# lc700x/desktop2stereo

Measured on AMD Instinct MI355X. Metric: stereo frames/sec @1080p DepthAnything-v2-ViT-B, higher is better.
Workload: dtype bf16; 1 GPU; DepthAnything-v2-vitb bf16, 1920x1080 uint8 RGB noise frames, batch 1 per GPU, Depth Resolution 518 (model input 294x518), Full-SBS uint8 output 3840x1080, pred; parallelism=frame-sharded dp1, no data-path collective (each rank generates its own frames)

## Files before the change

### desktop2stereo_amd/csrc/conv3.hip

```cpp
#include "conv3_tile.h"
#include <algorithm>

namespace d2s {

static_assert(sizeof(GemmA) + sizeof(GemmEpi) + 8 >= KERNARG_WARM_BYTES, "KERNARG_WARM reads past the kernarg segment");


template <int N_> __device__ __forceinline__ void c3_wait_vm() { asm volatile("s_waitcnt vmcnt(%0) lgkmcnt(0)" ::"n"(N_) : "memory"); }

template <int PST> __device__ __forceinline__ int c3_lane_pixel(int fr) {
    if constexpr ((PST & 1) == 0) return fr;
    else return fr < 4 ? 2 * fr : (fr < 12 ? 2 * (fr - 4) + 1 : 2 * (fr - 8));
}
template <int PST> __device__ __forceinline__ int c3_chunk_slot(int c) {
    if constexpr ((PST & 1) == 0) return c;
    else return (c & ~3) | ((c & 1) << 1) | ((c >> 1) & 1);
}

template <int CPP, int PST, int BN, int WM, int WN, int NS, int HG = 3 >
__global__ void __launch_bounds__(64 * WM * WN)
conv3_halo2_kernel(GemmA a, const bf16_t* __restrict__ W, int M, int N, int Kpad, GemmEpi e, int xn) {
    KERNARG_WARM(kaw_)
    KERNARG_WARM_END(kaw_)
    constexpr int TW = 16, TH = 8, HWD = TW + 2, HPX = (TH + 2) * HWD;
// ... 631 lines not shown
        c3_load_wfrags<64>(wf, W, N, Kpad, 0, fr, fg);
        c3_head_consts(e, N, fg, cb, cw);
        __syncthreads();
        int tn = walk.at(++kk);
        __syncthreads();
        const int cw4 = wid * 4;
        const int hb0 = (cw4 * HWD + fr) * PST + fg;
        int buf = 0;
        for (; t >= 0;) {
            f32x4 acc[4][2];
            const u32x4* hp = lds + buf * HALO + hb0;
            auto mma_rows = [&](auto r0c) {
                constexpr int R0 = decltype(r0c)::value;
                static_for<3>([&](auto rc) {
                    constexpr int r = R0 + decltype(rc)::value;
                    static_for<3>([&](auto kxc) {
                        constexpr int kx = decltype(kxc)::value;
#pragma unroll
                        for (int ks = 0; ks < 2; ++ks) {
                            const u32x4 fa = hp[(r * HWD + kx) * PST + ks * 4];
                            static_for<3>([&](auto kyc) {
                                constexpr int ky = 2 - decltype(kyc)::value;
                                constexpr int i = r - ky;
                                if constexpr (i >= 0 && i < 4) {
#pragma unroll
                                    for (int j = 0; j < 2; ++j) mma_chunk(acc[i][j], wf[ky * 3 + kx][ks][j], fa, bf16_t());
                                }
                            });
                        }
                    });
                });
            };
#pragma unroll
            for (int i = 0; i < 4; ++i)
#pragma unroll
                for (int j = 0; j < 2; ++j) acc[i][j] = (f32x4){0.f, 0.f, 0.f, 0.f};
            C3U_T(u0)
            mma_rows(std::integral_constant<int, 0>());
            C3U_T(u1)
            __syncthreads();
            C3U_T(u2)
            const int tnn = tn >= 0 ? walk.at(++kk) : -1;
            mma_rows(std::integral_constant<int, 3>());
            int b, ty0, tx0;
            tiles.org(t, b, ty0, tx0);
            float sr[4];
#pragma unroll
            for (int i = 0; i < 4; ++i) {
                float s = 0.f;
#pragma unroll
                for (int j = 0; j < 2; ++j) s += c3_head_dot(acc[i][j], cb[j], cw[j]);
                sr[i] = s;
            }
            typedef unsigned u2_ __attribute__((ext_vector_type(2)));
            const u2_ p01 = __builtin_amdgcn_permlane16_swap(__float_as_uint(sr[0]), __float_as_uint(sr[1]), false, false);
            const u2_ p23 = __builtin_amdgcn_permlane16_swap(__float_as_uint(sr[2]), __float_as_uint(sr[3]), false, false);
            const float c01 = __uint_as_float(p01[0]) + __uint_as_float(p01[1]);
            const float c23 = __uint_as_float(p23[0]) + __uint_as_float(p23[1]);
            const u2_ q = __builtin_amdgcn_permlane32_swap(__float_as_uint(c01), __float_as_uint(c23), false, false);
            const float sv = __uint_as_float(q[0]) + __uint_as_float(q[1]);
            {
                const int y = ty0 + cw4 + fg, x = tx0 + fr;
                if (y < a.Ho && x < a.Wo) ((float*)e.out)[((long)b * a.Ho + y) * a.Wo + x] = head_activation(sv + e.head_b3, e.head_max_depth);
            }
            if (VS < VU && tn >= 0) v_pass(tile_geo(tn), buf ^ 1, KS_(), KU_());
            C3U_T(u3)
            __syncthreads();
            C3U_T(u4)
            C3U_ACC(0, u1 - u0) C3U_ACC(1, u2 - u1) C3U_ACC(2, u3 - u2) C3U_ACC(3, u4 - u3) C3U_ACC(8, 1)
            buf ^= 1;
            t = tn; tn = tnn;
        }
    } else {
        TileGeo gn = tile_geo(t), gnn = gn;
        h_request(gn);
        h_compute();
        __syncthreads();
        int tn = walk.at(++kk);
        v_pass(gn, 0, K0_(), KU_());
        if (tn >= 0) { gn = tile_geo(tn); h_request(gn); }
        __syncthreads();
        int buf = 0;
        for (; t >= 0;) {
            C3U_T(u0)
            if (tn >= 0) h_compute();
            C3U_T(u1)
            __syncthreads();
            C3U_T(u2)
            const int tnn = tn >= 0 ? walk.at(++kk) : -1;
            if (tn >= 0) {
                if (tnn >= 0) { gnn = tile_geo(tnn); h_request(gnn); }
                v_pass(gn, buf ^ 1, K0_(), KS_());
                gn = gnn;
            }
            C3U_T(u3)
            __syncthreads();
            C3U_T(u4)
            C3U_ACC(4, u1 - u0) C3U_ACC(5, u2 - u1) C3U_ACC(6, u3 - u2) C3U_ACC(7, u4 - u3)
            buf ^= 1;
            t = tn; tn = tnn;
        }
    }
}

#ifdef D2S_C3_TIMING
__device__ unsigned long long c3_timing[256 * 8];
#define C3_T(var) const long var = wall_clock64();
#define C3_ACC(SLOT, expr) { if (threadIdx.x == 0 && blockIdx.x < 256) c3_timing[blockIdx.x * 8 + (SLOT)] += (unsigned long long)(expr); }
#else
#define C3_T(var) {}
#define C3_ACC(SLOT, expr) {}
#endif

template <int TH, int TW>
__global__ void __launch_bounds__(512)
conv3_wide_kernel(GemmA a, const bf16_t* __restrict__ W, int N, int Kpad, GemmEpi e, int ntiles) {
    KERNARG_WARM(kaw_)
    KERNARG_WARM_END(kaw_)
    constexpr int CPP = 16, PST = 17, HWD = TW + 2, HPX = (TH + 2) * HWD, HALO = HPX * PST;
    constexpr int NCH = HPX * CPP, NLD = (NCH + 511) / 512;
    constexpr int WN = 2, FM = 4, FN = 4, FPR = TW / 16;
    constexpr int NS = 8, WST = 128 * 4, NKT = 36, PD = NS - 1;
    constexpr int HKT = 28;
    static_assert(TH * TW == 256 && TW % 16 == 0, "256-pixel tiles of 16-pixel fragments");
    __shared__ __attribute__((aligned(16))) u32x4 lds[NS * WST + HALO];
    D2S_POISON_LDS(lds, NS * WST + HALO)
    u32x4* const halo = lds + NS * WST;

    const int tid = threadIdx.x, lane = tid & 63;
    const int wid = __builtin_amdgcn_readfirstlane(tid >> 6);
    const int wave_m = wid / WN, wave_n = wid % WN, grp = wid >> 2;
    const int fr = lane & 15, fg = lane >> 4, px = c3_lane_pixel<PST>(fr);
    const C3Tiles<TH, TW> tiles(a);
    const C3Walk<true> walk(ntiles);
    int kk = 0, t = walk.at(0);
    if (t < 0) return;

    const __amdgpu_buffer_rsrc_t rsW = __builtin_amdgcn_make_buffer_rsrc(uniform_ptr(W), 0, (unsigned)((long)((N + 255) / 256 * 256) * Kpad * 2), 0x00020000);
    auto wswz = [](int r) { const int k = (r >> 2) & 3; return (((k ^ (k >> 1)) & 1) << 1) | (k >> 1); };
    unsigned voW;
    {
        const int r = wid * 16 + (lane >> 2);
        voW = (unsigned)((long)r * Kpad * 2) + (unsigned)(((lane & 3) ^ wswz(r)) * 16);
    }
    auto issue_w = [&](int stage, int kt) { lds_dma16(rsW, lds + stage * WST + wid * 64, voW, kt * 64); };

    const int floor_ = relu_floor_bf16(a);
    u32x4 hr[NLD];
    auto load_halo = [&](int tt) {
        int b, ty0, tx0;
        tiles.org(tt, b, ty0, tx0);
        const bf16_t* img = (const bf16_t*)a.ptr + (long)b * a.Hi * a.Wi * a.C;
#pragma unroll
        for (int k = 0; k < NLD; ++k) {
            const int idx = tid + k * 512;
            const int p = idx >> 4, c = idx & 15;
            const int hy = p / HWD, hx = p - hy * HWD;
            int iy = ty0 + hy - 1, ix = tx0 + hx - 1;
            const bool in = idx < NCH && iy >= 0 && iy < a.Hi && ix >= 0 && ix < a.Wi;
            iy = in ? iy : 0; ix = in ? ix : 0;
            const u32x4 v = *(const u32x4*)(img + ((long)iy * a.Wi + ix) * a.C + c * 8);
            hr[k] = in ? v : (u32x4){0u, 0u, 0u, 0u};
        }
    };
    auto store_halo = [&]() {
#pragma unroll
        for (int k = 0; k < NLD; ++k) {
            const int idx = tid + k * 512;
            if (idx < NCH) halo[(idx >> 4) * PST + c3_chunk_slot<PST>(idx & 15)] = relu_frag(hr[k], floor_, bf16_t());
        }
    };

    const u32x4* hb[FM];
    int frow[FM], fcol[FM];
#pragma unroll
    for (int i = 0; i < FM; ++i) {
        const int f = wave_m * FM + i;
        frow[i] = f / FPR; fcol[i] = (f % FPR) * 16 + px;
        hb[i] = halo + (frow[i] * HWD + fcol[i]) * PST + c3_chunk_slot<PST>(fg);
    }
    int wro[FN];
#pragma unroll
    for (int jn = 0; jn < FN; ++jn) { const int r = wave_n * 64 + jn * 16 + fr; wro[jn] = r * 4 + (fg ^ wswz(r)); }

#pragma unroll
    for (int k = 0; k < PD - 1; ++k) issue_w(k, k);
    load_halo(t);
    store_halo();
    int gb = 0;
    C3_T(t_begin)
    while (t >= 0) {
        C3_T(t_a)
        const int tn = walk.at(++kk);
        const int tl = tn >= 0 ? tn : t;
        f32x4 acc[FM][FN];
#pragma unroll
        for (int i = 0; i < FM; ++i)
#pragma unroll
            for (int jn = 0; jn < FN; ++jn) acc[i][jn] = (f32x4){0.f, 0.f, 0.f, 0.f};
        u32x4 fa[2][FM], fb[2][FN];
        auto read_frags = [&](auto ktc, u32x4* fa_, u32x4* fb_) {
            constexpr int kt = decltype(ktc)::value;
            constexpr int tap = kt / 4, q = kt % 4, ky = tap / 3, kx = tap % 3;
            const u32x4* B_l = lds + ((gb + kt) & (NS - 1)) * WST;
#pragma unroll
            for (int jn = 0; jn < FN; ++jn) fb_[jn] = B_l[wro[jn]];
#pragma unroll
            for (int i = 0; i < FM; ++i) fa_[i] = hb[i][(ky * HWD + kx) * PST + q * 4];
        };
        c3_wait_vm<0>();
        __builtin_amdgcn_s_barrier();
        issue_w((gb + PD - 1) & (NS - 1), PD - 1);
        read_frags(std::integral_constant<int, 0>{}, fa[0], fb[0]);
        if (grp) __builtin_amdgcn_s_barrier();
        static_for<NKT>([&](auto ktc) {
            constexpr int kt = decltype(ktc)::value;
            __builtin_amdgcn_sched_barrier(0);
#pragma unroll
            for (int i = 0; i < FM; ++i)
#pragma unroll
                for (int jn = 0; jn < FN; ++jn) mma_chunk(acc[i][jn], fb[kt & 1][jn], fa[kt & 1][i], bf16_t());
            __builtin_amdgcn_sched_barrier(0);
            __builtin_amdgcn_s_barrier();
            if constexpr (kt < NKT - 1) {
                issue_w((gb + kt + PD) & (NS - 1), (kt + PD) % NKT);
                if constexpr (kt == HKT) load_halo(tl);
                read_frags(std::integral_constant<int, kt + 1>{}, fa[(kt + 1) & 1], fb[(kt + 1) & 1]);
                if constexpr (kt + 2 < NKT) {
                    if constexpr (kt >= HKT && kt <= HKT + PD - 2) asm volatile("s_waitcnt vmcnt(%0)" ::"n"(NLD + PD - 2) : "memory");
                    else asm volatile("s_waitcnt vmcnt(%0)" ::"n"(PD - 2) : "memory");
                }
            }
            __builtin_amdgcn_sched_barrier(0);
            __builtin_amdgcn_s_barrier();
#ifdef D2S_C3_TIMING
            if constexpr (kt == 0) { C3_ACC(4, wall_clock64() - t_a) }
#endif
        });
        if (!grp) __builtin_amdgcn_s_barrier();
        C3_T(t_b)
        C3_ACC(0, t_b - t_a)
        int b, ty0, tx0;
        tiles.org(t, b, ty0, tx0);
        bool ok[FM];
        long mo[FM];
        uint2 rr[FM][FN];
#pragma unroll
        for (int i = 0; i < FM; ++i) {
            const int y = ty0 + frow[i], x = tx0 + fcol[i];
            ok[i] = y < a.Ho && x < a.Wo;
            mo[i] = ok[i] ? ((long)(b * a.Ho + y) * a.Wo + x) * e.ldc + wave_n * 64 + fg * 4 : (long)(wave_n * 64 + fg * 4);
        }
        auto load_res = [&]() {
            const bf16_t* rp = (const bf16_t*)e.res1;
#pragma unroll
            for (int i = 0; i < FM; ++i)
#pragma unroll
                for (int jn = 0; jn < FN; ++jn) rr[i][jn] = *(const uint2*)(rp + mo[i] + jn * 16);
        };
        float cb[FN][4];
#pragma unroll
        for (int jn = 0; jn < FN; ++jn) {
            if (e.bias) load4(e.bias + wave_n * 64 + jn * 16 + fg * 4, cb[jn]);
            else cb[jn][0] = cb[jn][1] = cb[jn][2] = cb[jn][3] = 0.f;
        }
        if (e.res1) load_res();
        C3_T(t_c)
        C3_ACC(1, t_c - t_b)
        __builtin_amdgcn_s_waitcnt(0xc07f);
        __builtin_amdgcn_s_barrier();
        if (tn >= 0) store_halo();
        C3_T(t_d)
        C3_ACC(2, t_d - t_c)
#pragma unroll
        for (int i = 0; i < FM; ++i)
#pragma unroll
            for (int jn = 0; jn < FN; ++jn) {
                float v[4] = {acc[i][jn][0] + cb[jn][0], acc[i][jn][1] + cb[jn][1], acc[i][jn][2] + cb[jn][2], acc[i][jn][3] + cb[jn][3]};
                if (e.act == ACT_RELU) { v[0] = fmaxf(v[0], 0.f); v[1] = fmaxf(v[1], 0.f); v[2] = fmaxf(v[2], 0.f); v[3] = fmaxf(v[3], 0.f); }
                if (e.res1) {
                    const uint2 r = rr[i][jn];
                    v[0] += __uint_as_float(r.x << 16); v[1] += __uint_as_float(r.x & 0xffff0000u);
                    v[2] += __uint_as_float(r.y << 16); v[3] += __uint_as_float(r.y & 0xffff0000u);
                }
                if (ok[i]) *(uint2*)((bf16_t*)e.out + mo[i] + jn * 16) = make_uint2(pk_bf16(v[0], v[1]), pk_bf16(v[2], v[3]));
            }
        C3_ACC(6, wall_clock64() - t_d)
        C3_ACC(3, 1)
        gb = (gb + NKT) & (NS - 1); t = tn;
    }
    c3_wait_vm<0>();
    C3_ACC(5, wall_clock64() - t_begin)
}


struct RcuArgs {
    const bf16_t* x;
    bf16_t* out;
    const bf16_t *w1, *w2, *wp;
    const float *b1, *b2, *bp;
    int H, W, nimg, Kpad, KpadP;
};
constexpr int RCU_TH = 4, RCU_TW = 8;
typedef short s16x4 __attribute__((ext_vector_type(4)));
__device__ __forceinline__ uint2 rcu_pack4(const float v[4], bool relu) {
    uint2 t = make_uint2(pk_bf16(v[0], v[1]), pk_bf16(v[2], v[3]));
    if (relu) t = __builtin_bit_cast(uint2, __builtin_elementwise_max(__builtin_bit_cast(s16x4, t), (s16x4){0, 0, 0, 0}));
    return t;
}
typedef unsigned int u32x2 __attribute__((ext_vector_type(2)));
__device__ __forceinline__ void rcu_lds_write_b64(const u32x4* chunk, int half, uint2 v) {
    const unsigned addr = (unsigned)(unsigned long)((__attribute__((address_space(3))) const char*)chunk) + (unsigned)half * 8u;
    const u32x2 d = {v.x, v.y};
    asm volatile("ds_write_b64 %0, %1" ::"v"(addr), "v"(d) : "memory");
}
template <int PROJ>
__global__ void __launch_bounds__(512)
conv3_rcu_kernel(RcuArgs r) {
    constexpr int TH = RCU_TH, TW = RCU_TW, CPP = 16, PST = 17, NW = 8;
    constexpr int W0 = TW + 4, P0 = (TH + 4) * W0;
    constexpr int W1 = TW + 2, P1 = (TH + 2) * W1;
    constexpr int NKT = 18, NG = 2 * NKT + (PROJ ? 2 : 0);
    constexpr int WST = 128 * 8;
    constexpr int NS = 7, PD = NS - 1, BI = 128 / (8 * NW);
    static_assert(P1 <= 64 && TH * TW == 32 && BI == 2 && NG > PD, "fragment counts below are for a 4 x 8 tile");
    __shared__ __attribute__((aligned(16))) u32x4 lds[NS * WST + P0 * PST + P1 * PST];
    D2S_POISON_LDS(lds, NS * WST + P0 * PST + P1 * PST)
    u32x4* const h0 = lds + NS * WST;
    u32x4* const h1 = h0 + P0 * PST;
    u32x4* const h2 = h0;

    const int tid = threadIdx.x, lane = tid & 63;
    const int wid = __builtin_amdgcn_readfirstlane(tid >> 6);
    const int fr = lane & 15, fg = lane >> 4;
    GemmA a = {};
    a.ptr = r.x; a.Hi = a.Ho = r.H; a.Wi = a.Wo = r.W; a.C = 128; a.relu = 1;
    const C3Tiles<TH, TW> tiles(a);
    int b, ty0, tx0;
    tiles.org(blockIdx.x, b, ty0, tx0);

    const int n0 = wid * 16 + fg * 4;
    float c1[4], c2[4], cp[4] = {0.f, 0.f, 0.f, 0.f};
    load4(r.b1 + n0, c1); load4(r.b2 + n0, c2);
    if constexpr (PROJ) load4(r.bp + n0, cp);

    const unsigned wbytes = 256u * (unsigned)r.Kpad * 2u, pbytes = 256u * (unsigned)r.KpadP * 2u;
    const __amdgpu_buffer_rsrc_t rs1 = __builtin_amdgcn_make_buffer_rsrc(uniform_ptr(r.w1), 0, wbytes, 0x00020000);
    const __amdgpu_buffer_rsrc_t rs2 = __builtin_amdgcn_make_buffer_rsrc(uniform_ptr(r.w2), 0, wbytes, 0x00020000);
    const __amdgpu_buffer_rsrc_t rsP = __builtin_amdgcn_make_buffer_rsrc(uniform_ptr(PROJ ? r.wp : r.w2), 0, PROJ ? pbytes : wbytes, 0x00020000);
    unsigned voW[BI], voP[BI];
#pragma unroll
    for (int i = 0; i < BI; ++i) {
        const int row = (i * NW + wid) * 8 + (lane >> 3);
        const unsigned ch = (unsigned)(((lane & 7) ^ ((row >> 1) & 7)) * 16);
        voW[i] = (unsigned)(row * r.Kpad * 2) + ch;
        voP[i] = (unsigned)(row * r.KpadP * 2) + ch;
    }
    auto issue = [&](int g, int slot) {
        u32x4* st_ = lds + slot * WST;
        if (g < NKT) {
#pragma unroll
            for (int i = 0; i < BI; ++i) lds_dma16(rs1, st_ + (i * NW + wid) * 64, voW[i], g * 128);
        } else if (!PROJ || g < 2 * NKT) {
#pragma unroll
            for (int i = 0; i < BI; ++i) lds_dma16(rs2, st_ + (i * NW + wid) * 64, voW[i], (g - NKT) * 128);
        } else {
#pragma unroll
            for (int i = 0; i < BI; ++i) lds_dma16(rsP, st_ + (i * NW + wid) * 64, voP[i], (g - 2 * NKT) * 128);
        }
    };
#pragma unroll
    for (int t = 0; t < PD; ++t) issue(t, t);

    conv_halo_fill<bf16_t, 64 * NW, 3>(a, b, ty0 - 1, tx0 - 1, W0, P0, CPP, tid, h0,
        [&](int p, int c) { return p * PST + c; },
        [&](u32x4 v) { return relu_frag(v, relu_floor_bf16(a), bf16_t()); });
#pragma unroll
    for (int q = 0; q < 4; ++q) asm volatile("" : "+v"(c1[q]), "+v"(c2[q]), "+v"(cp[q]));

    int g = 0, slot = 0, islot = PD;
    auto ring_step = [&]() -> const u32x4* {
        const int rem = NG - 1 - g;
        if (rem >= PD - 1) c3_wait_vm<(PD - 1) * BI>();
        else if (rem == 4) c3_wait_vm<4 * BI>();
        else if (rem == 3) c3_wait_vm<3 * BI>();
        else if (rem == 2) c3_wait_vm<2 * BI>();
        else if (rem == 1) c3_wait_vm<1 * BI>();
        else c3_wait_vm<0>();
        __builtin_amdgcn_s_barrier();
        if (g + PD < NG) issue(g + PD, islot);
        const u32x4* B_l = lds + slot * WST;
        ++g;
        slot = slot + 1 == NS ? 0 : slot + 1;
        islot = islot + 1 == NS ? 0 : islot + 1;
        return B_l;
    };
    static_assert(PD == 6, "ring_step spells out the waits of the last PD - 1 tiles");
    int wo[2];
    {
        const int row = wid * 16 + fr;
#pragma unroll
        for (int ks = 0; ks < 2; ++ks) wo[ks] = row * 8 + ((ks * 4 + fg) ^ ((row >> 1) & 7));
    }

    {
        const u32x4* hb[4];
#pragma unroll
        for (int f = 0; f < 4; ++f) {
            const int p = f * 16 + fr < P1 ? f * 16 + fr : P1 - 1;
            hb[f] = h0 + ((p / W1) * W0 + p % W1) * PST + fg;
        }
        f32x4 acc[4];
#pragma unroll
        for (int f = 0; f < 4; ++f) acc[f] = (f32x4){0.f, 0.f, 0.f, 0.f};
#pragma unroll 1
        for (int kt = 0; kt < NKT; ++kt) {
            const int tap = kt >> 1, ky = (tap * 11) >> 5, kx = tap - 3 * ky;
            const int toff = (ky * W0 + kx) * PST + (kt & 1) * 8;
            const u32x4* B_l = ring_step();
            u32x4 fb[2], fa[2][4];
#pragma unroll
            for (int ks = 0; ks < 2; ++ks) {
                fb[ks] = B_l[wo[ks]];
#pragma unroll
                for (int f = 0; f < 4; ++f) fa[ks][f] = hb[f][toff + ks * 4];
            }
            __builtin_amdgcn_sched_barrier(0);
#pragma unroll
            for (int ks = 0; ks < 2; ++ks)
#pragma unroll
                for (int f = 0; f < 4; ++f) mma_chunk(acc[f], fb[ks], fa[ks][f], bf16_t());
        }
#pragma unroll
        for (int f = 0; f < 4; ++f) {
            const int p = f * 16 + fr;
            const int py = p / W1, px = p - py * W1;
            const int iy = ty0 - 1 + py, ix = tx0 - 1 + px;
            const float v[4] = {acc[f][0] + c1[0], acc[f][1] + c1[1], acc[f][2] + c1[2], acc[f][3] + c1[3]};
            uint2 t = rcu_pack4(v, true);
            if (!(iy >= 0 && iy < r.H && ix >= 0 && ix < r.W)) t = make_uint2(0u, 0u);
            if (p < P1) rcu_lds_write_b64(h1 + p * PST + 2 * wid + (fg >> 1), fg & 1, t);
        }
    }

    const int oy0 = fr >> 3, ox = fr & 7;
    uint2 rcu[2];
    {
        const u32x4* hb[2];
#pragma unroll
        for (int f = 0; f < 2; ++f) hb[f] = h1 + ((2 * f + oy0) * W1 + ox) * PST + fg;
        f32x4 acc[2];
#pragma unroll
        for (int f = 0; f < 2; ++f) acc[f] = (f32x4){0.f, 0.f, 0.f, 0.f};
#pragma unroll 1
        for (int kt = 0; kt < NKT; ++kt) {
            const int tap = kt >> 1, ky = (tap * 11) >> 5, kx = tap - 3 * ky;
            const int toff = (ky * W1 + kx) * PST + (kt & 1) * 8;
            const u32x4* B_l = ring_step();
            u32x4 fb[2], fa[2][2];
#pragma unroll
            for (int ks = 0; ks < 2; ++ks) {
                fb[ks] = B_l[wo[ks]];
#pragma unroll
                for (int f = 0; f < 2; ++f) fa[ks][f] = hb[f][toff + ks * 4];
            }
            __builtin_amdgcn_sched_barrier(0);
#pragma unroll
            for (int ks = 0; ks < 2; ++ks)
#pragma unroll
                for (int f = 0; f < 2; ++f) mma_chunk(acc[f], fb[ks], fa[ks][f], bf16_t());
        }
        float xr[2][4];
#pragma unroll
        for (int f = 0; f < 2; ++f) {
            const int y = ty0 + 2 * f + oy0, x = tx0 + ox;
            const bool ok = y < r.H && x < r.W;
            load4(r.x + ((long)(b * r.H + (ok ? y : 0)) * r.W + (ok ? x : 0)) * 128 + n0, xr[f]);
        }
#pragma unroll
        for (int f = 0; f < 2; ++f) {
            float v[4] = {acc[f][0] + c2[0], acc[f][1] + c2[1], acc[f][2] + c2[2], acc[f][3] + c2[3]};
            v[0] += xr[f][0]; v[1] += xr[f][1]; v[2] += xr[f][2]; v[3] += xr[f][3];
            rcu[f] = rcu_pack4(v, false);
        }
    }
    if constexpr (!PROJ) {
#pragma unroll
        for (int f = 0; f < 2; ++f) {
            const int y = ty0 + 2 * f + oy0, x = tx0 + ox;
            if (y < r.H && x < r.W) *(uint2*)(r.out + ((long)(b * r.H + y) * r.W + x) * 128 + n0) = rcu[f];
        }
    } else {
#pragma unroll
        for (int f = 0; f < 2; ++f) rcu_lds_write_b64(h2 + (f * 16 + fr) * PST + 2 * wid + (fg >> 1), fg & 1, rcu[f]);
        f32x4 acc[2];
#pragma unroll
        for (int f = 0; f < 2; ++f) acc[f] = (f32x4){0.f, 0.f, 0.f, 0.f};
#pragma unroll 1
        for (int kt = 0; kt < 2; ++kt) {
            const u32x4* B_l = ring_step();
#pragma unroll
            for (int ks = 0; ks < 2; ++ks) {
                const u32x4 fb = B_l[wo[ks]];
#pragma unroll
                for (int f = 0; f < 2; ++f) mma_chunk(acc[f], fb, h2[(f * 16 + fr) * PST + fg + kt * 8 + ks * 4], bf16_t());
            }
        }
#pragma unroll
        for (int f = 0; f < 2; ++f) {
            const int y = ty0 + 2 * f + oy0, x = tx0 + ox;
            const float v[4] = {acc[f][0] + cp[0], acc[f][1] + cp[1], acc[f][2] + cp[2], acc[f][3] + cp[3]};
            if (y < r.H && x < r.W) *(uint2*)(r.out + ((long)(b * r.H + y) * r.W + x) * 128 + n0) = rcu_pack4(v, false);
        }
    }
}

#define C3_INSTANCES(P, H, R)                                                                                                    \
    R(C3_RCU, conv3_rcu_kernel<0>)                                                                                               \
    R(C3_RCU_PROJ, conv3_rcu_kernel<1>)                                                                                          \
    P(C3_HEAD_UPS, conv3_head_ups_kernel)                                                                                        \
    P(C3_HEAD_1, conv3_head_kernel<1>)                                                                                           \
    P(C3_HEAD_0, conv3_head_kernel<0>)                                                                                           \
    P(C3_C128_UPS, conv3_c128_ups_kernel)                                                                                        \
    P(C3_WIDE_8_32, conv3_wide_kernel<8,32>)                                                                                     \
    P(C3_WIDE_16_16, conv3_wide_kernel<16,16>)                                                                                   \
    H(C3_H2_MID, 16,17,64,4,2,10,6)                                             \
    H(C3_H2_C128_N128, 16,17,128,2,4,2)                     \
    H(C3_H2_C128_N64, 16,17,64,4,2,3)                                                                                            \
    H(C3_H2_C128_N32, 16,17,32,4,1,3)                                                                                            \
    H(C3_H2_C64_N128, 8,10,128,2,4,3)                                                                                            \
    H(C3_H2_C64_N64, 8,10,64,4,2,3)                                                                                              \
    H(C3_H2_C64_N32, 8,10,32,4,1,3)
#define C3_ID(ID, ...) ID,
enum { C3_INSTANCES(C3_ID, C3_ID, C3_ID) };
#undef C3_ID
#define C3_BLOCK(CPP, PST, BN, WM, WN, ...) 64 * WM * WN
#define C3_P(ID, ...) {#__VA_ARGS__, 512},
#define C3_H(ID, ...) {"conv3_halo2_kernel<" #__VA_ARGS__ ">", C3_BLOCK(__VA_ARGS__)},
static const struct { const char* name; int block; } c3_inst[] = { C3_INSTANCES(C3_P, C3_H, C3_P) };
#undef C3_P
#undef C3_H
#undef C3_BLOCK
static void c3_plan(GemmPlan& p, int inst, unsigned grid, int xn, const GemmA& a) {
    p.family = GEMM_CONV3; p.inst = inst; p.name = c3_inst[inst].name; p.grid = grid; p.block = c3_inst[inst].block; p.xn = xn; p.ups = a.ups;
}


static bool c3_head_persistent_ok(const GemmA& a, int N, const GemmEpi& e, long t16) {
    static EnvInt headp_min{"D2S_HEADP_MIN", 2048};
    return e.map == MAP_HEAD && a.C == 64 && N <= 32 && t16 >= headp_min.get();
}
static bool c3_c128_ups_ok(const GemmA& a, int N, const GemmEpi& e, int nimg, long t8) {
    static EnvInt c128_min{"D2S_HEAD1P_MIN", 2048};
    return a.ups && a.C == 128 && N == 64 && e.map == MAP_ROWS && !a.relu && a.usy <= 0.5f && a.usx <= 0.5f && a.Hs >= 2 && a.Ws >= 2 &&
           (e.out_type == OUT_T || e.out_type == OUT_BF16) && !e.scale && !e.res1 && !e.res2 && e.act == ACT_NONE && !e.deq && !e.out2 && !(e.ldc & 7) &&
           c128_min.get() > 0 && t8 >= c128_min.get() && t8 < (1L << 30) && (long)nimg * a.Hs * a.Ws * a.C * 2 < (1L << 31);
}
static bool c3_wide_ok(const GemmA& a, int N, int Kpad, const GemmEpi& e, long t256, int ncu) {
    static EnvInt no_wide{"D2S_NO_WIDE", 0};
    return !no_wide.get() && !a.ups && e.map == MAP_ROWS && a.C == 128 && N == 128 && (long)gemm_npad(N) * Kpad * 2 < (1L << 31) &&
           (e.out_type == OUT_T || e.out_type == OUT_BF16) && !e.scale && !e.res2 && !e.res1_mod && (e.act == ACT_NONE || e.act == ACT_RELU) &&
           t256 >= 384 && t256 < (1L << 30) && (ncu & ~7) >= 8;
}
static bool c3_mid_ok(const GemmA& a, int N, int Kpad, const GemmEpi& e, long t8, int ncu) {
    return a.C == 128 && e.map == MAP_ROWS && N % 64 == 0 && (long)gemm_npad(N) * Kpad * 2 < (1L << 31) &&
           t8 * (N / 64) <= ncu && t8 * (N / 64) * 2 > ncu;
}

bool plan_conv3_halo2(const GemmA& a, int M, int N, int K, int Kpad, const GemmEpi& e, GemmPlan& p) {
    static EnvInt off{"D2S_NO_HALO2", 0};
    if (off.get()) return false;
    if (a.mode != A_CONV3 || a.stride != 1 || a.Hi != a.Ho || a.Wi != a.Wo || (a.C != 64 && a.C != 128) || K != 9 * a.C) return false;
    if (!(e.map == MAP_ROWS || e.map == MAP_HEAD) || e.rows_per_img || e.ln_stats || e.stats_out || e.deq || e.ksplit > 1) return false;
    if (e.map == MAP_HEAD && N > 32) return false;
    if (N != 32 && N != 64 && (N & 127)) return false;
    const int nimg = M / (a.Ho * a.Wo);
    if ((long)nimg * a.Ho * a.Wo != M) return false;
    const int ncu = device_cu_count();
    const long per16 = (long)cdiv(a.Ho, 16) * cdiv(a.Wo, 16), per8x32 = (long)cdiv(a.Ho, 8) * cdiv(a.Wo, 32);
    const long t16 = nimg * per16, t8 = (long)nimg * cdiv(a.Ho, 8) * cdiv(a.Wo, 16);
    const long t256 = nimg * std::min(per8x32, per16);
    if (c3_head_persistent_ok(a, N, e, t16)) {
        static EnvInt no_headups{"D2S_NO_HEADUPS", 0};
        if (a.ups && (no_headups.get() || a.usy > 0.6f || a.usx > 0.6f || a.relu)) return false;
        static EnvInt ups_v1{"D2S_HEADUPS_V1", 0};
        const bool ups_fits = (long)nimg * a.Hs * a.Ws * a.C * 2 < (1L << 31) && (long)a.Ws * a.C * 2 <= 65536;
        c3_plan(p, a.ups ? (!ups_v1.get() && ups_fits ? C3_HEAD_UPS : C3_HEAD_1) : C3_HEAD_0, std::min(ncu, (int)t16), (int)t16, a);
        return true;
    }
    if (c3_c128_ups_ok(a, N, e, nimg, t8)) {
        c3_plan(p, C3_C128_UPS, std::min(ncu & ~7, (int)t8), (int)t8, a);
        return true;
    }
    if (c3_wide_ok(a, N, Kpad, e, t256, ncu)) {
        c3_plan(p, per8x32 <= per16 ? C3_WIDE_8_32 : C3_WIDE_16_16, ncu & ~7, (int)t256, a);
        return true;
    }
    unsigned grid = 0;
    if (c3_mid_ok(a, N, Kpad, e, t8, ncu)) {
        const int xn = pick_xn((int)t8, N / 64, 64, Kpad, 2, grid);
        c3_plan(p, C3_H2_MID, grid, xn, a);
        return true;
    }
    const int bn = N <= 32 ? 32 : (N <= 64 ? 64 : 128);
    if (t8 * cdiv(N, bn) < 384) return false;
    if ((long)gemm_npad(N) * Kpad * 2 >= (1L << 31)) return false;
    const int xn = pick_xn((int)t8, cdiv(N, bn), bn, Kpad, 2, grid);
    if (a.C == 128) c3_plan(p, bn == 128 ? C3_H2_C128_N128 : (bn == 64 ? C3_H2_C128_N64 : C3_H2_C128_N32), grid, xn, a);
    else c3_plan(p, bn == 128 ? C3_H2_C64_N128 : (bn == 64 ? C3_H2_C64_N64 : C3_H2_C64_N32), grid, xn, a);
    return true;
}

void launch_conv3_halo2(const GemmPlan& p, const GemmA& a, const void* W, int M, int N, int Kpad, const GemmEpi& e, hipStream_t st) {
    const bf16_t* w = (const bf16_t*)W;
    const dim3 grid(p.grid), block(p.block);
    switch (p.inst) {
#define C3_P(ID, ...) case ID: hipLaunchKernelGGL((__VA_ARGS__), grid, block, 0, st, a, w, N, Kpad, e, p.xn); break;
#define C3_H(ID, ...) case ID: hipLaunchKernelGGL((conv3_halo2_kernel<__VA_ARGS__>), grid, block, 0, st, a, w, M, N, Kpad, e, p.xn); break;
#define C3_R(ID, ...) case ID: break;
        C3_INSTANCES(C3_P, C3_H, C3_R)
#undef C3_P
#undef C3_H
#undef C3_R
    }
}

bool c3_rcu_ok(bool plain_bf16, int C, int nimg, int H, int W) {
    return plain_bf16 && C == 128 && nimg > 0 && H > 0 && W > 0 && (long)nimg * H * W * 128 < (1L << 31) &&
           (long)nimg * cdiv(H, RCU_TH) * cdiv(W, RCU_TW) <= device_cu_count();
}
bool plan_conv3_rcu(bool plain_bf16, int C, int nimg, int H, int W, bool proj, GemmPlan& p) {
    if (!c3_rcu_ok(plain_bf16, C, nimg, H, W)) return false;
    p = GemmPlan{};
    const int inst = proj ? C3_RCU_PROJ : C3_RCU;
    p.family = GEMM_CONV3; p.inst = inst; p.name = c3_inst[inst].name; p.block = c3_inst[inst].block;
    p.grid = (unsigned)(nimg * cdiv(H, RCU_TH) * cdiv(W, RCU_TW)); p.ksplit = 1;
    return true;
}
void launch_conv3_rcu(const GemmPlan& p, const RcuOp& o, hipStream_t st) {
    const RcuArgs r = {(const bf16_t*)o.x, (bf16_t*)o.out, (const bf16_t*)o.w1, (const bf16_t*)o.w2, (const bf16_t*)o.wp, o.b1, o.b2, o.bp,
                       o.H, o.W, o.nimg, o.Kpad, o.KpadP};
    const dim3 grid(p.grid), block(p.block);
    switch (p.inst) {
#define C3_N(ID, ...)
#define C3_R(ID, ...) case ID: hipLaunchKernelGGL((__VA_ARGS__), grid, block, 0, st, r); break;
        C3_INSTANCES(C3_N, C3_N, C3_R)
#undef C3_N
#undef C3_R
    }
    kernel_note() = KernelNote{p.name, 0, 1, NOTE_TAIL_NONE};
}

}

#ifdef D2S_C3U_TIMING
extern "C" int d2s_c3u_timing(unsigned long long* out, int clear) {
    if (out) D2S_HIP(hipMemcpyFromSymbol(out, HIP_SYMBOL(d2s::c3u_timing), sizeof(unsigned long long) * 256 * 9));
    if (clear) { static unsigned long long z[256 * 9]; D2S_HIP(hipMemcpyToSymbol(HIP_SYMBOL(d2s::c3u_timing), z, sizeof(z))); }
    return D2S_OK;
}
#endif
#ifdef D2S_C3_TIMING
extern "C" int d2s_c3_timing(unsigned long long* out, int clear) {
    if (out) D2S_HIP(hipMemcpyFromSymbol(out, HIP_SYMBOL(d2s::c3_timing), sizeof(unsigned long long) * 256 * 8));
    if (clear) { static unsigned long long z[256 * 8]; D2S_HIP(hipMemcpyToSymbol(HIP_SYMBOL(d2s::c3_timing), z, sizeof(z))); }
    return D2S_OK;
}
#endif
```

### desktop2stereo_amd/csrc/core.cpp

```cpp
#include "common.h"

#include <atomic>
#include <cstdlib>

namespace d2s {

static thread_local std::string g_err;

void set_error(const std::string& msg) { g_err = msg; }

int hip_fail(hipError_t err, const char* what, const char* file, int line) {
    g_err = std::string("HIP error ") + hipGetErrorName(err) + " (" + hipGetErrorString(err) + ") in " + what +
            " at " + file + ":" + std::to_string(line);
    return D2S_E_HIP;
}

int env_int(const char* name, int dflt) {
    const char* v = getenv(name);
    return v ? atoi(v) : dflt;
}

static std::atomic<int> g_env_gen{1};
int env_generation() { return g_env_gen.load(std::memory_order_relaxed); }
int EnvInt::get() {
    const uint32_t g = (uint32_t)env_generation();
    const uint64_t c = cached.load(std::memory_order_relaxed);
    if ((uint32_t)(c >> 32) == g) return (int)(uint32_t)c;
    const int val = env_int(name, dflt);
    cached.store(((uint64_t)g << 32) | (uint32_t)val, std::memory_order_relaxed);
    return val;
}

int device_cu_count() {
    static const int n = [] { hipDeviceProp_t p; int d = 0; (void)hipGetDevice(&d); return hipGetDeviceProperties(&p, d) == hipSuccess ? p.multiProcessorCount : 256; }();
    return n;
}

}

extern "C" int d2s_debug_lds_poison(void) {
#ifdef D2S_LDS_POISON
    return 1;
#else
    return 0;
#endif
}
extern "C" int d2s_debug_reload_env(void) { return d2s::g_env_gen.fetch_add(1) + 1; }
extern "C" const char* d2s_last_error(void) { return d2s::g_err.c_str(); }
extern "C" int d2s_version(void) { return 129; }
```

Measured before the change: 916.8 stereo frames/s.

## Make RCU weight ring wave-private to drop per-step barriers; pad LDS halos

The RCU conv kernel now has each wave DMA exactly the weight rows it later reads. That lets the per-k-step s_barrier in the ring be removed, keeping only three block-wide barriers at the phase boundaries between conv1, conv2 and the projection. The halo LDS layout gains a row pitch and a pixel stride of 18. The lane-to-pixel mapping is rearranged, with compile-time checks that the A-fragment reads are bank-conflict free and that every halo position has exactly one owner. The goal is to cut barrier stalls and LDS bank conflicts, at the cost of relying on per-wave vmcnt ordering for correctness and a slightly larger LDS footprint.

```diff
diff --git a/desktop2stereo_amd/csrc/conv3.hip b/desktop2stereo_amd/csrc/conv3.hip
--- a/desktop2stereo_amd/csrc/conv3.hip
+++ b/desktop2stereo_amd/csrc/conv3.hip
@@ -957,6 +957,58 @@
     int H, W, nimg, Kpad, KpadP;
 };
 constexpr int RCU_TH = 4, RCU_TW = 8;
+constexpr int RCU_PST = 18;
+constexpr int RCU_W0 = RCU_TW + 4, RCU_W1 = RCU_TW + 2;
+constexpr int RCU_RP0 = RCU_W0 * RCU_PST + 12;
+constexpr int RCU_RP1 = RCU_W1 * RCU_PST;
+__host__ __device__ constexpr int rcu_half(int fr) { return fr >= 4 && fr < 12; }
+__host__ __device__ constexpr int rcu_idx(int fr) { return fr < 4 ? fr : (fr < 12 ? fr - 4 : fr - 8); }
+__host__ __device__ constexpr int rcu_c1_row(int f, int fr) { return f < 3 ? 2 * f + rcu_half(fr) : (rcu_idx(fr) >> 1) + 2 * rcu_half(fr); }
+__host__ __device__ constexpr int rcu_c1_col(int f, int fr) { return f < 3 ? rcu_idx(fr) : 8 + (rcu_idx(fr) & 1); }
+__host__ __device__ constexpr bool rcu_c1_owns(int f, int fr) { return f < 3 || !(rcu_half(fr) && rcu_idx(fr) < 4); }
+struct RcuSlots { int s[64]; };
+constexpr int rcu_b128_cycles(const RcuSlots& t) {
+    int cyc = 0;
+    for (int g = 0; g < 4; ++g) {
+        int n[16] = {}, worst = 0;
+        for (int lane = 0; lane < 64; ++lane) {
+            const int l = lane & 31;
+            const int grp = 2 * (lane >> 5) + ((l < 4 || (l >= 12 && l < 16) || (l >= 20 && l < 28)) ? 0 : 1);
+            if (grp != g) continue;
+            const int c = ++n[t.s[lane] & 15];
+            worst = c > worst ? c : worst;
+        }
+        cyc += worst;
+    }
+    return cyc;
+}
+constexpr RcuSlots rcu_slots(int region, int f) {
+    RcuSlots t{};
+    for (int lane = 0; lane < 64; ++lane) {
+        const int fr = lane & 15, fg = lane >> 4;
+        t.s[lane] = fg + (region == 0 ? rcu_c1_row(f, fr) * RCU_RP0 + rcu_c1_col(f, fr) * RCU_PST
+                        : region == 1 ? (2 * f + rcu_half(fr)) * RCU_RP1 + rcu_idx(fr) * RCU_PST
+                                      : (16 * f + fr) * RCU_PST);
+    }
+    return t;
+}
+constexpr bool rcu_c1_covers() {
+    int n[6 * RCU_W1] = {};
+    for (int f = 0; f < 4; ++f)
+        for (int fr = 0; fr < 16; ++fr) {
+            const int row = rcu_c1_row(f, fr), col = rcu_c1_col(f, fr);
+            if (row < 0 || row >= 6 || col < 0 || col >= RCU_W1) return false;
+            if (rcu_c1_owns(f, fr)) ++n[row * RCU_W1 + col];
+        }
+    for (int p = 0; p < 6 * RCU_W1; ++p)
+        if (n[p] != 1) return false;
+    return true;
+}
+static_assert(rcu_c1_covers(), "conv1's lanes must own every ring-extended position once");
+static_assert(rcu_b128_cycles(rcu_slots(0, 0)) == 4 && rcu_b128_cycles(rcu_slots(0, 1)) == 4 && rcu_b128_cycles(rcu_slots(0, 2)) == 4 &&
+              rcu_b128_cycles(rcu_slots(0, 3)) == 4, "conv1's A-fragment reads must be conflict-free");
+static_assert(rcu_b128_cycles(rcu_slots(1, 0)) == 4 && rcu_b128_cycles(rcu_slots(1, 1)) == 4, "conv2's A-fragment reads must be conflict-free");
+static_assert(rcu_b128_cycles(rcu_slots(2, 0)) == 4 && rcu_b128_cycles(rcu_slots(2, 1)) == 4, "the projection's A-fragment reads must be conflict-free");
 typedef short s16x4 __attribute__((ext_vector_type(4)));
 __device__ __forceinline__ uint2 rcu_pack4(const float v[4], bool relu) {
     uint2 t = make_uint2(pk_bf16(v[0], v[1]), pk_bf16(v[2], v[3]));
@@ -972,17 +1024,19 @@
 template <int PROJ>
 __global__ void __launch_bounds__(512)
 conv3_rcu_kernel(RcuArgs r) {
-    constexpr int TH = RCU_TH, TW = RCU_TW, CPP = 16, PST = 17, NW = 8;
-    constexpr int W0 = TW + 4, P0 = (TH + 4) * W0;
-    constexpr int W1 = TW + 2, P1 = (TH + 2) * W1;
+    constexpr int TH = RCU_TH, TW = RCU_TW, CPP = 16, PST = RCU_PST, NW = 8;
+    constexpr int W0 = RCU_W0, P0 = (TH + 4) * W0, RP0 = RCU_RP0;
+    constexpr int W1 = RCU_W1, P1 = (TH + 2) * W1, RP1 = RCU_RP1;
+    constexpr int L0 = (TH + 4) * RP0, L1 = (TH + 2) * RP1;
     constexpr int NKT = 18, NG = 2 * NKT + (PROJ ? 2 : 0);
     constexpr int WST = 128 * 8;
     constexpr int NS = 7, PD = NS - 1, BI = 128 / (8 * NW);
     static_assert(P1 <= 64 && TH * TW == 32 && BI == 2 && NG > PD, "fragment counts below are for a 4 x 8 tile");
-    __shared__ __attribute__((aligned(16))) u32x4 lds[NS * WST + P0 * PST + P1 * PST];
-    D2S_POISON_LDS(lds, NS * WST + P0 * PST + P1 * PST)
+    static_assert(TH * TW * PST <= L0 && (NS * WST + L0 + L1) * 16 <= 160 * 1024, "h2 lies over h0; one block's LDS");
+    __shared__ __attribute__((aligned(16))) u32x4 lds[NS * WST + L0 + L1];
+    D2S_POISON_LDS(lds, NS * WST + L0 + L1)
     u32x4* const h0 = lds + NS * WST;
-    u32x4* const h1 = h0 + P0 * PST;
+    u32x4* const h1 = h0 + L0;
     u32x4* const h2 = h0;
 
     const int tid = threadIdx.x, lane = tid & 63;
@@ -1006,7 +1060,7 @@
     unsigned voW[BI], voP[BI];
 #pragma unroll
     for (int i = 0; i < BI; ++i) {
-        const int row = (i * NW + wid) * 8 + (lane >> 3);
+        const int row = (wid * BI + i) * 8 + (lane >> 3);
         const unsigned ch = (unsigned)(((lane & 7) ^ ((row >> 1) & 7)) * 16);
         voW[i] = (unsigned)(row * r.Kpad * 2) + ch;
         voP[i] = (unsigned)(row * r.KpadP * 2) + ch;
@@ -1015,23 +1069,28 @@
         u32x4* st_ = lds + slot * WST;
         if (g < NKT) {
 #pragma unroll
-            for (int i = 0; i < BI; ++i) lds_dma16(rs1, st_ + (i * NW + wid) * 64, voW[i], g * 128);
+            for (int i = 0; i < BI; ++i) lds_dma16(rs1, st_ + (wid * BI + i) * 64, voW[i], g * 128);
         } else if (!PROJ || g < 2 * NKT) {
 #pragma unroll
-            for (int i = 0; i < BI; ++i) lds_dma16(rs2, st_ + (i * NW + wid) * 64, voW[i], (g - NKT) * 128);
+            for (int i = 0; i < BI; ++i) lds_dma16(rs2, st_ + (wid * BI + i) * 64, voW[i], (g - NKT) * 128);
         } else {
 #pragma unroll
-            for (int i = 0; i < BI; ++i) lds_dma16(rsP, st_ + (i * NW + wid) * 64, voP[i], (g - 2 * NKT) * 128);
+            for (int i = 0; i < BI; ++i) lds_dma16(rsP, st_ + (wid * BI + i) * 64, voP[i], (g - 2 * NKT) * 128);
         }
     };
 #pragma unroll
     for (int t = 0; t < PD; ++t) issue(t, t);
 
     conv_halo_fill<bf16_t, 64 * NW, 3>(a, b, ty0 - 1, tx0 - 1, W0, P0, CPP, tid, h0,
-        [&](int p, int c) { return p * PST + c; },
+        [&](int p, int c) { return (p / W0) * RP0 + (p % W0) * PST + c; },
         [&](u32x4 v) { return relu_frag(v, relu_floor_bf16(a), bf16_t()); });
 #pragma unroll
     for (int q = 0; q < 4; ++q) asm volatile("" : "+v"(c1[q]), "+v"(c2[q]), "+v"(cp[q]));
+    auto seam = [&]() {
+        asm volatile("s_waitcnt lgkmcnt(0)" ::: "memory");
+        __builtin_amdgcn_s_barrier();
+    };
+    seam();
 
     int g = 0, slot = 0, islot = PD;
     auto ring_step = [&]() -> const u32x4* {
@@ -1042,7 +1101,6 @@
         else if (rem == 2) c3_wait_vm<2 * BI>();
         else if (rem == 1) c3_wait_vm<1 * BI>();
         else c3_wait_vm<0>();
-        __builtin_amdgcn_s_barrier();
         if (g + PD < NG) issue(g + PD, islot);
         const u32x4* B_l = lds + slot * WST;
         ++g;
@@ -1061,17 +1119,14 @@
     {
         const u32x4* hb[4];
 #pragma unroll
-        for (int f = 0; f < 4; ++f) {
-            const int p = f * 16 + fr < P1 ? f * 16 + fr : P1 - 1;
-            hb[f] = h0 + ((p / W1) * W0 + p % W1) * PST + fg;
-        }
+        for (int f = 0; f < 4; ++f) hb[f] = h0 + rcu_c1_row(f, fr) * RP0 + rcu_c1_col(f, fr) * PST + fg;
         f32x4 acc[4];
 #pragma unroll
         for (int f = 0; f < 4; ++f) acc[f] = (f32x4){0.f, 0.f, 0.f, 0.f};
 #pragma unroll 1
         for (int kt = 0; kt < NKT; ++kt) {
             const int tap = kt >> 1, ky = (tap * 11) >> 5, kx = tap - 3 * ky;
-            const int toff = (ky * W0 + kx) * PST + (kt & 1) * 8;
+            const int toff = ky * RP0 + kx * PST + (kt & 1) * 8;
             const u32x4* B_l = ring_step();
             u32x4 fb[2], fa[2][4];
 #pragma unroll
@@ -1088,29 +1143,29 @@
         }
 #pragma unroll
         for (int f = 0; f < 4; ++f) {
-            const int p = f * 16 + fr;
-            const int py = p / W1, px = p - py * W1;
+            const int py = rcu_c1_row(f, fr), px = rcu_c1_col(f, fr);
             const int iy = ty0 - 1 + py, ix = tx0 - 1 + px;
             const float v[4] = {acc[f][0] + c1[0], acc[f][1] + c1[1], acc[f][2] + c1[2], acc[f][3] + c1[3]};
             uint2 t = rcu_pack4(v, true);
             if (!(iy >= 0 && iy < r.H && ix >= 0 && ix < r.W)) t = make_uint2(0u, 0u);
-            if (p < P1) rcu_lds_write_b64(h1 + p * PST + 2 * wid + (fg >> 1), fg & 1, t);
-        }
-    }
-
-    const int oy0 = fr >> 3, ox = fr & 7;
+            if (rcu_c1_owns(f, fr)) rcu_lds_write_b64(h1 + py * RP1 + px * PST + 2 * wid + (fg >> 1), fg & 1, t);
+        }
+    }
+    seam();
+
+    const int oy0 = rcu_half(fr), ox = rcu_idx(fr);
     uint2 rcu[2];
     {
         const u32x4* hb[2];
 #pragma unroll
-        for (int f = 0; f < 2; ++f) hb[f] = h1 + ((2 * f + oy0) * W1 + ox) * PST + fg;
+        for (int f = 0; f < 2; ++f) hb[f] = h1 + (2 * f + oy0) * RP1 + ox * PST + fg;
         f32x4 acc[2];
 #pragma unroll
         for (int f = 0; f < 2; ++f) acc[f] = (f32x4){0.f, 0.f, 0.f, 0.f};
 #pragma unroll 1
         for (int kt = 0; kt < NKT; ++kt) {
             const int tap = kt >> 1, ky = (tap * 11) >> 5, kx = tap - 3 * ky;
-            const int toff = (ky * W1 + kx) * PST + (kt & 1) * 8;
+            const int toff = ky * RP1 + kx * PST + (kt & 1) * 8;
             const u32x4* B_l = ring_step();
             u32x4 fb[2], fa[2][2];
 #pragma unroll
@@ -1148,6 +1203,7 @@
     } else {
 #pragma unroll
         for (int f = 0; f < 2; ++f) rcu_lds_write_b64(h2 + (f * 16 + fr) * PST + 2 * wid + (fg >> 1), fg & 1, rcu[f]);
+        seam();
         f32x4 acc[2];
 #pragma unroll
         for (int f = 0; f < 2; ++f) acc[f] = (f32x4){0.f, 0.f, 0.f, 0.f};
diff --git a/desktop2stereo_amd/csrc/core.cpp b/desktop2stereo_amd/csrc/core.cpp
--- a/desktop2stereo_amd/csrc/core.cpp
+++ b/desktop2stereo_amd/csrc/core.cpp
@@ -47,4 +47,4 @@
 }
 extern "C" int d2s_debug_reload_env(void) { return d2s::g_env_gen.fetch_add(1) + 1; }
 extern "C" const char* d2s_last_error(void) { return d2s::g_err.c_str(); }
-extern "C" int d2s_version(void) { return 129; }
+extern "C" int d2s_version(void) { return 130; }
```

New measurement: 934.2 stereo frames/s, median of 6. +1.9%, better.
